# Ameek94/BOBE

Measured on AMD Instinct MI355X. Metric: GP fit+acquisition cycles/sec at N=4096 d=8, 65536 cands; Cholesky GF/s, higher is better.
Workload: dtype f64

## Files before the change

bobe_amd/csrc/gemm_f64.hpp:

```cpp
#pragma once
#include <hip/hip_runtime.h>
#include <stdint.h>
#include <type_traits>

namespace bobe {

typedef double v4d __attribute__((ext_vector_type(4)));
typedef double v2d __attribute__((ext_vector_type(2)));

constexpr int TILE = 128;
constexpr int TK = 16;
constexpr int GEMM_THREADS = 256;

enum Layout { KC = 0, RC = 1 };

template <int L, int R, int BK>
struct Img {
  static constexpr int stride = (L == KC) ? (BK + 2) : (R + 16);
  static constexpr int doubles = (L == KC) ? R * (BK + 2) : BK * (R + 16);
};
constexpr int imax(int a, int b) { return a > b ? a : b; }
template <int TM, int TN, int BK>
constexpr int gemm_smem_doubles() {
  return 2 * (imax(Img<KC, TM, BK>::doubles, Img<RC, TM, BK>::doubles) +
// ... 22 lines not shown
__device__ __forceinline__ void stage_load(v2d (&reg)[R * BK / 512], const double* __restrict__ p, int64_t ld,
                                           int64_t r0, int64_t k0, int t) {
  if (L == KC) {
    constexpr int VPR = BK / 2;
    const int kq = t % VPR;
    const int r = t / VPR;
#pragma unroll
    for (int i = 0; i < R * BK / 512; ++i)
      reg[i] = *reinterpret_cast<const v2d*>(p + (r0 + r + (256 / VPR) * i) * ld + k0 + 2 * kq);
  } else {
    constexpr int VPR = R / 2;
    const int c = t % VPR;
    const int k = t / VPR;
#pragma unroll
    for (int i = 0; i < R * BK / 512; ++i)
      reg[i] = *reinterpret_cast<const v2d*>(p + (k0 + k + (256 / VPR) * i) * ld + r0 + 2 * c);
  }
}

template <int L, int R, int BK>
__device__ __forceinline__ void stage_store(const v2d (&reg)[R * BK / 512], double* img, int t) {
  if (L == KC) {
    constexpr int VPR = BK / 2;
    const int kq = t % VPR;
    const int r = t / VPR;
#pragma unroll
    for (int i = 0; i < R * BK / 512; ++i)
      *reinterpret_cast<v2d*>(img + (r + (256 / VPR) * i) * (BK + 2) + 2 * kq) = reg[i];
  } else {
    constexpr int VPR = R / 2;
    const int c = t % VPR;
    const int k = t / VPR;
#pragma unroll
    for (int i = 0; i < R * BK / 512; ++i)
      *reinterpret_cast<v2d*>(img + (k + (256 / VPR) * i) * (R + 16) + 2 * c) = reg[i];
  }
}

template <int L, int R, int BK>
__device__ __forceinline__ double frag_read(const double* img, int woff, int s, int ks, int lane) {
  if (L == KC)
    return img[(woff + 16 * s + (lane & 15)) * (BK + 2) + 4 * ks + (lane >> 4)];
  else
    return img[(4 * ks + (lane >> 4)) * (R + 16) + woff + 16 * s + (lane & 15)];
}

template <int FM, int FN>
__device__ __forceinline__ void acc_zero(v4d (&acc)[FM][FN]) {
#pragma unroll
  for (int i = 0; i < FM; ++i)
#pragma unroll
    for (int j = 0; j < FN; ++j) acc[i][j] = (v4d){0.0, 0.0, 0.0, 0.0};
}

struct WgSync {
  __device__ __forceinline__ void sync() { __syncthreads(); }
};

template <int LA, int LB, int TM = 128, int TN = 128, int BK = BK128, bool NEGA = false, class SYNC = WgSync, bool TRIL = false>
__device__ __forceinline__ void gemm_tile(v4d (&acc)[TM / 32][TN / 32], const double* __restrict__ A, int64_t lda,
                                          int64_t m0, const double* __restrict__ B, int64_t ldb, int64_t n0,
                                          int64_t kbeg, int64_t kend, double* smem, int tid = threadIdx.x,
                                          SYNC* sy = nullptr) {
  WgSync wg_default;
  constexpr int FM = TM / 32, FN = TN / 32;
  constexpr int IA = Img<LA, TM, BK>::doubles;
  constexpr int IB = Img<LB, TN, BK>::doubles;
  const int t = tid;
  const int lane = t & 63;
  const int wave = t >> 6;
  const int wm = (wave >> 1) * (TM / 2);
  const int wn = (wave & 1) * (TN / 2);
  if (kend <= kbeg) return;
  v2d ra[TM * BK / 512], rb[TN * BK / 512];
  stage_load<LA, TM, BK>(ra, A, lda, m0, kbeg, t);
  stage_load<LB, TN, BK>(rb, B, ldb, n0, kbeg, t);
  stage_store<LA, TM, BK>(ra, smem, t);
  stage_store<LB, TN, BK>(rb, smem + IA, t);
  if (sy) sy->sync(); else wg_default.sync();
  int buf = 0;
  const int wmu = TRIL ? __builtin_amdgcn_readfirstlane(wm) : 0;
  auto kstep = [&](int64_t k0, auto in_c, int rel) {
    constexpr bool IN = decltype(in_c)::value;
    const bool more = (k0 + BK) < kend;
    if (more) {
      stage_load<LA, TM, BK>(ra, A, lda, m0, k0 + BK, t);
      stage_load<LB, TN, BK>(rb, B, ldb, n0, k0 + BK, t);
    }
    const double* ia = smem + buf * (IA + IB);
    const double* ib = ia + IA;
#pragma unroll
    for (int ks = 0; ks < BK / 4; ++ks) {
      double a[FM], b[FN];
#pragma unroll
      for (int s = 0; s < FM; ++s) {
        a[s] = frag_read<LA, TM, BK>(ia, wm, s, ks, lane);
        if (NEGA) a[s] = -a[s];
      }
#pragma unroll
      for (int s = 0; s < FN; ++s) b[s] = frag_read<LB, TN, BK>(ib, wn, s, ks, lane);
#pragma unroll
      for (int i = 0; i < FM; ++i) {
        if (IN && rel + 4 * ks > wmu + 16 * i + 15) continue;
#pragma unroll
        for (int j = 0; j < FN; ++j)
          acc[i][j] = __builtin_amdgcn_mfma_f64_16x16x4f64(a[i], b[j], acc[i][j], 0, 0, 0);
      }
    }
    if (more) {
      double* na = smem + (buf ^ 1) * (IA + IB);
      stage_store<LA, TM, BK>(ra, na, t);
      stage_store<LB, TN, BK>(rb, na + IA, t);
    }
    if (sy) sy->sync(); else wg_default.sync();
    buf ^= 1;
  };
  const int64_t kd = TRIL ? (kend - TM > kbeg ? kend - TM : kbeg) : kend;
  for (int64_t k0 = kbeg; k0 < kd; k0 += BK) kstep(k0, std::false_type(), 0);
  if (TRIL)
    for (int64_t k0 = kd; k0 < kend; k0 += BK) kstep(k0, std::true_type(), (int)(k0 - (kend - TM)));
}

template <int TM = 128>
__device__ __forceinline__ int acc_row(int i, int r, int tid = threadIdx.x) {
  const int t = tid;
  return ((t >> 6) >> 1) * (TM / 2) + 16 * i + ((t & 63) >> 4) + 4 * r;
}
template <int TN = 128>
__device__ __forceinline__ int acc_col(int j, int tid = threadIdx.x) {
  const int t = tid;
  return ((t >> 6) & 1) * (TN / 2) + 16 * j + (t & 15);
}

template <int TM = 128, int TN = 128>
__device__ __forceinline__ void store_tile(const v4d (&acc)[TM / 32][TN / 32], double* __restrict__ C, int64_t ldc,
                                           int64_t m0, int64_t n0, double alpha, double beta, int tid = threadIdx.x) {
#pragma unroll
  for (int i = 0; i < TM / 32; ++i)
#pragma unroll
    for (int j = 0; j < TN / 32; ++j)
#pragma unroll
      for (int r = 0; r < 4; ++r) {
        double* q = C + (m0 + acc_row<TM>(i, r, tid)) * ldc + n0 + acc_col<TN>(j, tid);
        double v = alpha * acc[i][j][r];
        if (beta != 0.0) v += beta * (*q);
        *q = v;
      }
}

template <int TM = 128, int TN = 128>
__device__ __forceinline__ void load_tile(v4d (&acc)[TM / 32][TN / 32], const double* __restrict__ C, int64_t ldc,
                                          int64_t m0, int64_t n0, int tid = threadIdx.x) {
#pragma unroll
  for (int i = 0; i < TM / 32; ++i)
#pragma unroll
    for (int j = 0; j < TN / 32; ++j)
#pragma unroll
      for (int r = 0; r < 4; ++r) acc[i][j][r] = C[(m0 + acc_row<TM>(i, r, tid)) * ldc + n0 + acc_col<TN>(j, tid)];
}

__device__ __forceinline__ void tri_decode(int t, int& i, int& j) {
  int ii = (int)((sqrt(8.0 * (double)t + 1.0) - 1.0) * 0.5);
  while ((ii + 1) * (ii + 2) / 2 <= t) ++ii;
  while (ii * (ii + 1) / 2 > t) --ii;
  i = ii;
  j = t - ii * (ii + 1) / 2;
}

__device__ __forceinline__ int xcd_share(int b, int per) { return per > 0 ? (b & 7) * per + (b >> 3) : b; }

__device__ __forceinline__ void tri_grouped(int t, int n, int& i, int& j) {
  int ii, jj;
  tri_decode(t, ii, jj);
// ... 27 lines not shown
```

bobe_amd/csrc/gp_factor.hip:

```cpp
#include "gp_handle.hpp"

#include <chrono>

#include "chol_kernels.hpp"

using namespace bobe;

namespace bobe {

constexpr int SYRK32_BK = 128, SYRK64_BK = 16;
constexpr int SYRK32_SMEM = gemm_smem_doubles_exact<KC, KC, 32, 32, SYRK32_BK>() * 8 / 2;
constexpr int SYRK64_SMEM = gemm_smem_doubles_exact<KC, KC, 64, 64, SYRK64_BK>() * 8;

void configure_factor_kernels() {
  static bool done[64] = {false};
  int dev = 0;
  HIPCHK(hipGetDevice(&dev));
  if (dev < 0 || dev >= 64 || done[dev]) return;
  allow_big_lds(k_potf2<true>, POTF2_SMEM_BYTES);
  allow_big_lds(k_potf2<false>, POTF2_SMEM_BYTES);
  allow_big_lds(k_trti_diag, POTF2_SMEM_BYTES);
  allow_big_lds(k_trsm_panel, TRSM_SMEM_BYTES);
  allow_big_lds((k_chol_panel<false, 3>), POTF2_SMEM_BYTES);
  allow_big_lds((k_chol_panel<false, 4>), POTF2_SMEM_BYTES);
  allow_big_lds((k_chol_panel<true, 3>), POTF2_SMEM_BYTES);
  allow_big_lds((k_chol_panel<true, 4>), POTF2_SMEM_BYTES);
  allow_big_lds(k_trtri_T<128>, GEMM_SMEM_BYTES);
  allow_big_lds(k_trtri_R<128>, GEMM_SMEM_BYTES);
  allow_big_lds(k_syrk_trail<64, SYRK64_BK>, SYRK64_SMEM);
  allow_big_lds(k_syrk_trail<32, SYRK32_BK>, SYRK32_SMEM);
  allow_big_lds(k_trtri_T<64>, GEMM64_SMEM_BYTES);
  allow_big_lds(k_trtri_R<64>, GEMM64_SMEM_BYTES);
  allow_big_lds(k_trtri_T<32>, GEMM32_SMEM_BYTES);
  allow_big_lds(k_trtri_R<32>, GEMM32_SMEM_BYTES);
  allow_big_lds(k_lauum_tiles32, GEMM32_SMEM_BYTES);
  allow_big_lds(k_lauum_grad<0, 8, 64>, GEMM64_SMEM_BYTES);
  allow_big_lds(k_lauum_grad<0, 16, 64>, GEMM64_SMEM_BYTES);
  allow_big_lds(k_lauum_grad<0, 32, 64>, GEMM64_SMEM_BYTES);
  allow_big_lds(k_lauum_grad<1, 8, 64>, GEMM64_SMEM_BYTES);
  allow_big_lds(k_lauum_grad<1, 16, 64>, GEMM64_SMEM_BYTES);
  allow_big_lds(k_lauum_grad<1, 32, 64>, GEMM64_SMEM_BYTES);
  allow_big_lds(k_lauum_grad<0, 8, 128>, GEMM_SMEM_BYTES);
  allow_big_lds(k_lauum_grad<0, 16, 128>, GEMM_SMEM_BYTES);
  allow_big_lds(k_lauum_grad<0, 32, 128>, GEMM_SMEM_BYTES);
  allow_big_lds(k_lauum_grad<1, 8, 128>, GEMM_SMEM_BYTES);
  allow_big_lds(k_lauum_grad<1, 16, 128>, GEMM_SMEM_BYTES);
  allow_big_lds(k_lauum_grad<1, 32, 128>, GEMM_SMEM_BYTES);
  done[dev] = true;
}

const Tuning& tuning() {
  static Tuning t = [] {
    Tuning v{512, 600, 300, 1, BOBE_MAX_MLL_SLOTS, 2048, 1, 1, false, false, true};
    auto geti = [](const char* name, int& dst) {
      const char* e = std::getenv(name);
      if (e) dst = std::atoi(e);
      return e != nullptr;
    };
    geti("BOBE_SYRK32_BELOW", v.syrk32_below);
    geti("BOBE_TRTRI64", v.trtri64_below);
    geti("BOBE_PAIR_MIN", v.pair_min);
    geti("BOBE_LOCKSTEP_MIN_N", v.lockstep_min_n);
    v.mll_slots_set = geti("BOBE_MLL_SLOTS", v.mll_slots);
    geti("BOBE_GRAPH_MAX_N", v.graph_max_n);
    geti("BOBE_XCD_SHARES", v.xcd_shares);
    geti("BOBE_FILL", v.fill);
    v.trace = std::getenv("BOBE_TRACE") != nullptr;
    int reuse = 1;
    geti("BOBE_FACTOR_REUSE", reuse);
    v.factor_reuse = reuse != 0;
    return v;
  }();
  return t;
}

double default_refine_kappa() {
  static const double v = [] {
    const char* e = std::getenv("BOBE_REFINE_KAPPA");
    return e ? std::atof(e) : 1e6;
  }();
  return v;
}

int default_solve_block() {
  static const int v = [] {
    const char* e = std::getenv("BOBE_SOLVE_BLOCK");
    const int b = e ? std::atoi(e) : TILE;
    return b > 0 ? (b + TILE - 1) / TILE * TILE : TILE;
  }();
  return v;
}

int default_solve_panel() {
  static const int v = [] {
    const char* e = std::getenv("BOBE_SOLVE_PANEL");
    const int b = e ? std::atoi(e) : 512;
    return b > 0 ? (b + TILE - 1) / TILE * TILE : 512;
  }();
  return v;
}

int64_t default_solve_chunk() {
  static const int64_t v = [] {
    const char* e = std::getenv("BOBE_SOLVE_CHUNK");
    const int64_t c = e ? std::atoll(e) : 32768;
    return c > 0 ? (c + TILE - 1) / TILE * TILE : 0;
  }();
  return v;
}

double default_pivot_floor_ulp() {
  static const double v = [] {
    const char* e = std::getenv("BOBE_PIVOT_FLOOR_ULP");
    if (!e) return 0.0;
    const double u = std::atof(e);
    return u >= 0.0 ? u : 0.0;
  }();
  return v;
}

}

void bobe_gp::build_probs() {
// ... 1129 lines not shown
```

bobe_amd/csrc/gp_handle.hpp:

```cpp
#pragma once
#include "../../include/bobe_gp.h"

#include <hip/hip_runtime.h>

#include <algorithm>
#include <array>
#include <climits>
#include <cmath>
#include <cstdio>
#include <cstdlib>
#include <cstring>
#include <map>
#include <mutex>
#include <stdexcept>
#include <string>
#include <vector>

#include "gemm_f64.hpp"
#include "gp_types.hpp"

namespace bobe {

struct Err : std::runtime_error {
  int code;
// ... 12 lines not shown

#define LAUNCH_CHECK() HIPCHK(hipGetLastError())

inline int64_t round_up(int64_t x, int64_t m) { return (x + m - 1) / m * m; }

inline bool is_device_ptr(const void* p) {
  if (!p) return false;
  hipPointerAttribute_t attr;
  hipError_t e = hipPointerGetAttributes(&attr, p);
  if (e != hipSuccess) {
    (void)hipGetLastError();
    return false;
  }
  return attr.type == hipMemoryTypeDevice || attr.type == hipMemoryTypeManaged;
}

struct DBuf {
  void* p = nullptr;
  size_t bytes = 0;
  void ensure(size_t b) {
    if (b <= bytes) return;
    if (p) HIPCHK(hipFree(p));
    p = nullptr;
    bytes = 0;
    HIPCHK(hipMalloc(&p, b));
    bytes = b;
  }
  void release() {
    if (p) (void)hipFree(p);
    p = nullptr;
    bytes = 0;
  }
  double* d() const { return static_cast<double*>(p); }
};

inline double pivot_floor(const Hyper& h, double ulp) {
  const double f = ulp * 2.220446049250313e-16 * (h.kvar + h.noise);
  return f < 0.25 ? f : 0.25;
}
inline bool pivots_resolved(double min_diag, double floor) { return min_diag * min_diag >= floor; }
double default_pivot_floor_ulp();
double default_refine_kappa();
int default_solve_block();
int default_solve_panel();
int64_t default_solve_chunk();

template <typename K>
void allow_big_lds(K kernel, int bytes) {
  HIPCHK(hipFuncSetAttribute(reinterpret_cast<const void*>(kernel), hipFuncAttributeMaxDynamicSharedMemorySize, bytes));
}

struct Tuning {
  int syrk32_below, trtri64_below, pair_min, lockstep_min_n, mll_slots, graph_max_n, xcd_shares, fill;
  bool mll_slots_set, trace, factor_reuse;
};
const Tuning& tuning();

constexpr int LAUUM64_BELOW = 1200;
constexpr int FILL_NEAR = 2;
constexpr int FILL_CHUNK = 3;
constexpr int FILL_SLACK = 16;
constexpr int FILL_PHASE = 1024;

struct TileGrid { int grid, per; };
inline TileGrid tile_grid(int ntiles) {
  if (!tuning().xcd_shares || ntiles < 256) return {ntiles, 0};
  const int per = (ntiles + 7) / 8;
  return {8 * per, per};
}

void configure_factor_kernels();
void configure_sweep_kernels();
void configure_consumer_kernels();

struct Depth { int first, count, nblocks; };

struct EvalTag {
  bool pending = false;
  bool valid = false;
  Hyper h;
  uint64_t gen = 0;
  int64_t Np = 0;
  int info = 0;
  double min_diag = 0.0;
  void arm(const Hyper& hh, uint64_t g, int64_t np) {
    valid = false;
    pending = true;
    h = hh;
    gen = g;
    Np = np;
  }
  void collected(const double* hr) {
    if (!pending) return;
    pending = false;
    valid = true;
    std::memcpy(&info, hr + 100, sizeof(int));
    min_diag = hr[101];
  }
  void clear() { pending = valid = false; }
};
inline bool same_hyper(const Hyper& a, const Hyper& b) {
  if (a.d != b.d || a.kern != b.kern || a.d < 0 || a.d > MAX_D) return false;
  return std::memcmp(a.ls, b.ls, (size_t)a.d * sizeof(double)) == 0 && std::memcmp(&a.kvar, &b.kvar, sizeof(double)) == 0 &&
         std::memcmp(&a.noise, &b.noise, sizeof(double)) == 0;
}

}
// ... 250 lines not shown
```

bobe_amd/csrc/gp_sweep.hip:

```cpp
#include "gp_handle.hpp"

#include "sweep_kernels.hpp"

using namespace bobe;

namespace bobe {
void configure_sweep_kernels() {
  static bool done[64] = {false};
  int dev = 0;
  HIPCHK(hipGetDevice(&dev));
  if (dev < 0 || dev >= 64 || done[dev]) return;
  allow_big_lds(k_trimul, GEMM_SMEM_BYTES);
  allow_big_lds(k_trimul_t, GEMM_SMEM_BYTES);
  allow_big_lds(k_trimul_v64, GEMM64_SMEM_BYTES);
  allow_big_lds(k_trimul_t64, GEMM64_SMEM_BYTES);
  allow_big_lds(k_blk_step, GEMM_SMEM_BYTES);
  allow_big_lds(k_cross_vv<128>, GEMM_SMEM_BYTES);
  allow_big_lds(k_cross_vv<64>, GEMM64_SMEM_BYTES);
  done[dev] = true;
}
}

void bobe_gp::decide_refinement(double min_diag) {
  const double piv = min_diag * min_diag;
  refine_v = refine_kappa >= 0.0 && piv > 0.0 && (hyp.kvar + hyp.noise) / piv > refine_kappa;
}

void bobe_gp::solve_v(double* B, int64_t ldb, int64_t ncp, double* V, int64_t ldv, double* qp, int64_t ldq) {
  if (!refine_v) {
    hipLaunchKernelGGL(k_trimul, dim3((unsigned)(ncp / TILE), (unsigned)nb), dim3(256), GEMM_SMEM_BYTES, stream,
                       (const double*)Linv.d(), Np, nb, (const double*)B, ldb, V, ldv, qp, ldq, (const double*)nullptr,
                       (int64_t)0, 0, (double*)nullptr, (int64_t)0);
    return;
  }
  if (!V) throw Err(BOBE_ERR_STATE, "solve_v: the blocked substitution needs a buffer for V");
  const int bt = std::max(1, solve_block / TILE);
  const int pt = std::max(bt, (int)(solve_panel / TILE) / bt * bt);
  const double* Lf = A.d();
  const double* Li = Linv.d();
  auto step = [&](int u_r0, int u_rows, int u_k0, int u_k1, int s_r0, int s_rows) {
    hipLaunchKernelGGL(k_blk_step, dim3((unsigned)(ncp / TILE), (unsigned)(u_rows + s_rows)), dim3(256), GEMM_SMEM_BYTES,
                       stream, Lf, Li, Np, B, ldb, V, ldv, qp, ldq, u_r0, u_rows, u_k0, u_k1, s_r0, s_rows);
  };
  for (int p0 = 0; p0 < nb; p0 += pt) {
    const int p1 = std::min(nb, p0 + pt);
    if (p0 > 0) step(p0, p1 - p0, 0, p0, 0, 0);
    for (int t0 = p0; t0 < p1; t0 += bt) {
      const int t1 = std::min(p1, t0 + bt);
      step(0, 0, 0, 0, t0, t1 - t0);
      if (t1 < p1) step(t1, p1 - t1, t0, t1, 0, 0);
    }
  }
}

void bobe_gp::prepare_z(const double* Z, int64_t M, int64_t Mp, bool need_w) {
  const bool host_z = !is_device_ptr(Z);
  const bool few = (Mp / TILE) * nb < 2 * std::max(num_cus, 1);
  auto make_w = [&]() {
    if (few)
      hipLaunchKernelGGL(k_trimul_t64, dim3((unsigned)(Mp / 64), (unsigned)(2 * nb)), dim3(256), GEMM64_SMEM_BYTES, stream,
                         (const double*)Linv.d(), Np, 2 * nb, (const double*)VZ.d(), Mp, WZ.d(), Mp);
    else
      hipLaunchKernelGGL(k_trimul_t, dim3((unsigned)(Mp / TILE), (unsigned)nb), dim3(256), GEMM_SMEM_BYTES, stream,
                         (const double*)Linv.d(), Np, nb, (const double*)VZ.d(), Mp, WZ.d(), Mp);
    LAUNCH_CHECK();
    wz_ready = true;
  };
  if (host_z && z_seen_m == M && std::memcmp(z_seen.data(), Z, (size_t)M * d * sizeof(double)) == 0) {
    if (need_w && !wz_ready) make_w();
    return;
  }
  forget_z();
  if (host_z) z_seen.assign(Z, Z + (size_t)M * d);
  const double* zin = fetch(Z, (size_t)M * d, z_stage);
  ZsT.ensure((size_t)d * Mp * sizeof(double));
  kXZ.ensure((size_t)Np * Mp * sizeof(double));
  VZ.ensure((size_t)Np * Mp * sizeof(double));
  WZ.ensure((size_t)Np * Mp * sizeof(double));
  basez.ensure((size_t)Mp * sizeof(double));
  qpart.ensure((size_t)2 * nb * (Mp > chunk ? Mp : chunk) * sizeof(double));
  scale(zin, M, Mp, hyp, ZsT.d(), Mp);
  kernel_matrix_cross(XsT.d(), Np, N, Np, ZsT.d(), Mp, M, Mp, hyp, kXZ.d(), Mp);
  if (refine_v) {
    solve_v(kXZ.d(), Mp, Mp, VZ.d(), Mp, qpart.d(), Mp);
    hipLaunchKernelGGL(k_predict_finalize, dim3((unsigned)((Mp + 255) / 256)), dim3(256), 0, stream,
                       (const double*)qpart.d(), Mp, nb, Mp, hyp.kvar + hyp.noise, 0, basez.d(), (double*)nullptr);
  } else if (few) {
    const int nt = 2 * nb;
    hipLaunchKernelGGL(k_trimul_v64, dim3((unsigned)(Mp / 64), (unsigned)nt), dim3(256), GEMM64_SMEM_BYTES, stream,
                       (const double*)Linv.d(), Np, nt, (const double*)kXZ.d(), Mp, VZ.d(), Mp, qpart.d(), Mp);
    hipLaunchKernelGGL(k_predict_finalize, dim3((unsigned)((Mp + 255) / 256)), dim3(256), 0, stream,
                       (const double*)qpart.d(), Mp, nt, Mp, hyp.kvar + hyp.noise, 0, basez.d(), (double*)nullptr);
  } else {
    hipLaunchKernelGGL(k_trimul, dim3((unsigned)(Mp / TILE), (unsigned)nb), dim3(256), GEMM_SMEM_BYTES, stream,
                       (const double*)Linv.d(), Np, nb, (const double*)kXZ.d(), Mp, VZ.d(), Mp, qpart.d(), Mp,
                       (const double*)nullptr, (int64_t)0, 0, (double*)nullptr, (int64_t)0);
    hipLaunchKernelGGL(k_predict_finalize, dim3((unsigned)((Mp + 255) / 256)), dim3(256), 0, stream,
                       (const double*)qpart.d(), Mp, nb, Mp, hyp.kvar + hyp.noise, 0, basez.d(), (double*)nullptr);
  }
  LAUNCH_CHECK();
  if (need_w) make_w();
  if (host_z) z_seen_m = M;
}

void bobe_gp::sweep(const double* cand, int64_t C, const double* Z, int64_t M, double y_std, double* wipv,
                    double* wipstd, double* mean, double* var, int policy, int64_t* argmin_v, double* min_v,
                    int64_t* argmin_s, double* min_s, double* fantasy_out, bool gated) {
  if (!factored) throw Err(BOBE_ERR_STATE, "call bobe_gp_factor first");
  if (C <= 0) throw Err(BOBE_ERR_ARG, "C must be positive");
  const bool do_wip = (Z != nullptr);
  if (do_wip && M <= 0) throw Err(BOBE_ERR_ARG, "M must be positive");
  const int64_t Mp = do_wip ? round_up(M, TILE) : 0;
  const int nzt = (int)(Mp / TILE);
  const double kself = hyp.kvar + hyp.noise;
  const bool need_v = wipv || argmin_v || min_v;
  const bool need_s = wipstd || argmin_s || min_s;
  const double* cin = fetch(cand, (size_t)C * d, in_stage);
  if (do_wip) prepare_z(Z, M, Mp, false);
  const int64_t CH = (refine_v && solve_chunk > 0 && !chunk_set) ? solve_chunk : chunk;
  bool cand_is_z = false;
  if (do_wip && C == M && C <= CH && !mean && !var) {
    if (is_device_ptr(cand) || is_device_ptr(Z)) cand_is_z = (cand == Z);
    else cand_is_z = std::memcmp(cand, Z, (size_t)C * d * sizeof(double)) == 0;
  }
  const int64_t SC = round_up(std::min<int64_t>(C, std::max<int64_t>(CH, 65536)), CH);
  CsT.ensure((size_t)d * SC * sizeof(double));
  if (!cand_is_z) kXC.ensure((size_t)Np * CH * sizeof(double));
  sc.ensure((size_t)SC * sizeof(double));
  qpart.ensure((size_t)nb * (Mp > CH ? Mp : CH) * sizeof(double));
  part.ensure((size_t)nb * (Np > CH ? Np : CH) * sizeof(double));
  if (do_wip) pv.ensure((size_t)Mp * SC * sizeof(double));
  if ((do_wip || refine_v) && !cand_is_z) vxc.ensure((size_t)Np * CH * sizeof(double));
  const bool fuse_cross = do_wip && !refine_v && C > CH;
  if (fuse_cross) vxc2.ensure((size_t)Np * CH * sizeof(double));
  double* vbuf[2] = {vxc.d(), fuse_cross ? vxc2.d() : vxc.d()};
  int vsel = 0;
  struct { bool valid; const double* V; int64_t ncp; double* cross; } pend = {false, nullptr, 0, nullptr};
  auto cross_alone = [&](const double* Vc, int64_t ncp_, double* cross_out, int64_t ldvc) {
    prof_begin(BOBE_PROF_CROSSVV);
    if ((int64_t)nzt * (ncp_ / TILE) >= 2 * std::max(num_cus, 1))
      hipLaunchKernelGGL(k_cross_vv<128>, dim3((unsigned)(ncp_ / TILE), (unsigned)nzt), dim3(256), GEMM_SMEM_BYTES, stream,
                         (const double*)VZ.d(), Mp, Vc, ldvc, Np, cross_out, SC);
    else
      hipLaunchKernelGGL(k_cross_vv<64>, dim3((unsigned)(ncp_ / 64), (unsigned)(Mp / 64)), dim3(256), GEMM64_SMEM_BYTES,
                         stream, (const double*)VZ.d(), Mp, Vc, ldvc, Np, cross_out, SC);
    prof_end(BOBE_PROF_CROSSVV);
  };
  double* d_mean = out_dev(mean, C, o_mean);
  double* d_var = out_dev(var, C, o_var);
  double* d_wipv = nullptr;
  double* d_wipstd = nullptr;
  if (do_wip) {
    if (need_v) {
      if (wipv) d_wipv = out_dev(wipv, C, o_wipv);
      else { o_wipv.ensure(C * sizeof(double)); d_wipv = o_wipv.d(); }
    }
    if (need_s) {
      if (wipstd) d_wipstd = out_dev(wipstd, C, o_wipstd);
      else { o_wipstd.ensure(C * sizeof(double)); d_wipstd = o_wipstd.d(); }
    }
  }
  double* d_fant = nullptr;
  if (fantasy_out) {
    d_fant = is_device_ptr(fantasy_out) ? fantasy_out : (kout.ensure((size_t)C * M * sizeof(double)), kout.d());
  }
  const int dcap = d <= 8 ? 8 : (d <= 16 ? 16 : 32);
  for (int64_t s0 = 0; s0 < C; s0 += SC) {
    const int64_t ns = (C - s0 < SC) ? (C - s0) : SC;
    const int64_t nsp = round_up(ns, TILE);
    scale(cin + s0 * d, ns, nsp, hyp, CsT.d(), SC);
    for (int64_t c0 = 0; c0 < ns; c0 += CH) {
      const int64_t nc = (ns - c0 < CH) ? (ns - c0) : CH;
      const int64_t ncp = round_up(nc, TILE);
      if (cand_is_z) {
        hipLaunchKernelGGL(k_colsq_tile_parts, dim3((unsigned)((ncp + 255) / 256), (unsigned)nb), dim3(256), 0, stream,
                           (const double*)VZ.d(), Mp, ncp, qpart.d(), CH);
        cross_alone(VZ.d(), ncp, pv.d() + c0, Mp);
        hipLaunchKernelGGL(k_predict_finalize, dim3((unsigned)((nc + 255) / 256)), dim3(256), 0, stream,
                           (const double*)qpart.d(), CH, nb, nc, kself, policy, sc.d() + c0, (double*)nullptr);
        LAUNCH_CHECK();
        continue;
      }
      prof_begin(BOBE_PROF_KXC);
      kernel_matrix_cross(XsT.d(), Np, N, Np, CsT.d() + c0, SC, nc, ncp, hyp, kXC.d(), CH,
                          d_mean ? (const double*)alpha.d() : nullptr, d_mean ? part.d() : nullptr, CH);
      prof_end(BOBE_PROF_KXC);
      if (d_mean) {
        hipLaunchKernelGGL(k_colsum_parts, dim3((unsigned)((nc + 255) / 256)), dim3(256), 0, stream,
                           (const double*)part.d(), CH, nb, 0, nc, d_mean + s0 + c0);
      }
      if (do_wip || d_var) {
        double* vcur = vbuf[vsel];
        prof_begin(BOBE_PROF_TRIMUL);
        if (fuse_cross) {
          const int ncv = (int)(ncp / TILE), ncx = pend.valid ? (int)(pend.ncp / TILE) : 0;
          const int nz = pend.valid ? nzt : 0;
          hipLaunchKernelGGL(k_trimul, dim3((unsigned)std::max(ncv, ncx), (unsigned)(nb + nz)), dim3(256), GEMM_SMEM_BYTES,
                             stream, (const double*)Linv.d(), Np, nb, (const double*)kXC.d(), CH, vcur, CH, qpart.d(), CH,
                             (const double*)VZ.d(), Mp, nz, pend.cross, SC, pend.V, CH, ncx, ncv);
          pend = {true, vcur, ncp, pv.d() + c0};
          vsel ^= 1;
        } else {
          solve_v(kXC.d(), CH, ncp, (do_wip || refine_v) ? vcur : nullptr, CH, qpart.d(), CH);
        }
        prof_end(BOBE_PROF_TRIMUL);
        if (do_wip && !fuse_cross) cross_alone(vcur, ncp, pv.d() + c0, CH);
        hipLaunchKernelGGL(k_predict_finalize, dim3((unsigned)((nc + 255) / 256)), dim3(256), 0, stream,
                           (const double*)qpart.d(), CH, nb, nc, kself, policy, sc.d() + c0,
                           d_var ? d_var + s0 + c0 : nullptr);
      }
      LAUNCH_CHECK();
    }
    if (pend.valid) {
      cross_alone(pend.V, pend.ncp, pend.cross, CH);
      pend.valid = false;
    }
    if (do_wip) {
      const dim3 grid((unsigned)((ns + 63) / 64));
      const size_t sm = (size_t)(d + 1) * 128 * sizeof(double);
      double* vo = d_fant ? d_fant + s0 * M : nullptr;
      prof_begin(BOBE_PROF_CROSS);
#define WS(KE, DC)                                                                                              \
  hipLaunchKernelGGL((k_wip_score<KE, DC>), grid, dim3(256), sm, stream, (const double*)pv.d(), SC,             \
                     (const double*)CsT.d(), SC, (const double*)ZsT.d(), Mp, M, (const double*)sc.d(),          \
                     (const double*)basez.d(), ns, hyp, y_std * y_std, d_wipv ? d_wipv + s0 : nullptr,          \
                     d_wipstd ? d_wipstd + s0 : nullptr, vo, M)
      if (hyp.kern == 0) {
        if (dcap == 8) WS(0, 8); else if (dcap == 16) WS(0, 16); else WS(0, 32);
      } else {
        if (dcap == 8) WS(1, 8); else if (dcap == 16) WS(1, 16); else WS(1, 32);
      }
#undef WS
      prof_end(BOBE_PROF_CROSS);
      LAUNCH_CHECK();
    }
  }
  if (gated && gate_on(gate) && (d_mean || d_var)) gate_apply(cin, C, nullptr, nullptr, d_mean, d_var, nullptr, nullptr);
  o_misc.ensure(8 * sizeof(double));
  double* m_val = o_misc.d();
  int64_t* m_idx = reinterpret_cast<int64_t*>(o_misc.d() + 2);
  const bool want_v = do_wip && (argmin_v || min_v);
  const bool want_s = do_wip && (argmin_s || min_s);
  if (want_v) hipLaunchKernelGGL(k_argmin, dim3(1), dim3(1024), 0, stream, (const double*)d_wipv, C, m_val, m_idx);
  if (want_s)
    hipLaunchKernelGGL(k_argmin, dim3(1), dim3(1024), 0, stream, (const double*)d_wipstd, C, m_val + 1, m_idx + 1);
  LAUNCH_CHECK();
  out_finish(mean, C, o_mean);
  out_finish(var, C, o_var);
  if (do_wip) {
    out_finish(wipv, C, o_wipv);
// ... 380 lines not shown
```

bobe_amd/csrc/sweep_kernels.hpp:

```cpp
#pragma once
#include "kernels_common.hpp"

namespace bobe {

__global__ __launch_bounds__(256, 2) void k_trimul(const double* __restrict__ Linv, int64_t ldi, int nb,
                                                   const double* __restrict__ B, int64_t ldb, double* __restrict__ V,
                                                   int64_t ldv, double* __restrict__ qpart, int64_t ldq,
                                                   const double* __restrict__ VZ, int64_t ldw, int nzt,
                                                   double* __restrict__ crossT, int64_t ldx,
                                                   const double* __restrict__ Bx = nullptr, int64_t ldbx = 0, int ncx = 0,
                                                   int ncv = 1 << 30) {
  extern __shared__ double smem[];
  const int tc = blockIdx.x;
  v4d acc[4][4];
  acc_zero(acc);
  if ((int)blockIdx.y < nzt) {
    if (tc >= ncx) return;
    const int tz = blockIdx.y;
    gemm_tile<RC, RC>(acc, VZ, ldw, (int64_t)tz * TILE, Bx, ldbx, (int64_t)tc * TILE, 0, (int64_t)nb * TILE, smem);
    store_tile(acc, crossT, ldx, (int64_t)tz * TILE, (int64_t)tc * TILE, 1.0, 0.0);
    return;
  }
  if (tc >= ncv) return;
  const int ti = nb - 1 - ((int)blockIdx.y - nzt);
  gemm_tile<KC, RC, TILE, TILE, BK128, false, WgSync, true>(acc, Linv, ldi, (int64_t)ti * TILE, B, ldb, (int64_t)tc * TILE, 0,
                                                            (int64_t)(ti + 1) * TILE, smem);
  if (V) store_tile(acc, V, ldv, (int64_t)ti * TILE, (int64_t)tc * TILE, 1.0, 0.0);
  if (qpart) {
    const int t = threadIdx.x, lane = t & 63, wave = t >> 6;
    double* red = smem;
#pragma unroll
    for (int j = 0; j < 4; ++j) {
      double s = 0.0;
#pragma unroll
      for (int i = 0; i < 4; ++i)
#pragma unroll
        for (int r = 0; r < 4; ++r) s += acc[i][j][r] * acc[i][j][r];
      s += __shfl_xor(s, 16, 64);
      s += __shfl_xor(s, 32, 64);
      if (lane < 16) red[(wave >> 1) * TILE + (wave & 1) * 64 + 16 * j + lane] = s;
    }
    __syncthreads();
    if (t < TILE) qpart[(int64_t)ti * ldq + (int64_t)tc * TILE + t] = red[t] + red[TILE + t];
  }
}

__global__ __launch_bounds__(256, 2) void k_blk_step(const double* __restrict__ L, const double* __restrict__ Linv,
                                                     int64_t ld, double* __restrict__ B, int64_t ldb,
                                                     double* __restrict__ V, int64_t ldv, double* __restrict__ qpart,
                                                     int64_t ldq, int u_r0, int u_rows, int u_k0, int u_k1, int s_r0,
                                                     int s_rows) {
  extern __shared__ double smem[];
  const int tc = blockIdx.x;
  v4d acc[4][4];
  acc_zero(acc);
  if ((int)blockIdx.y < u_rows) {
    const int ti = u_r0 + (int)blockIdx.y;
    gemm_tile<KC, RC>(acc, L, ld, (int64_t)ti * TILE, V, ldv, (int64_t)tc * TILE, (int64_t)u_k0 * TILE,
                      (int64_t)u_k1 * TILE, smem);
    store_tile(acc, B, ldb, (int64_t)ti * TILE, (int64_t)tc * TILE, -1.0, 1.0);
    return;
  }
  const int ti = s_r0 + s_rows - 1 - ((int)blockIdx.y - u_rows);
  gemm_tile<KC, RC, TILE, TILE, BK128, false, WgSync, true>(acc, Linv, ld, (int64_t)ti * TILE, B, ldb, (int64_t)tc * TILE,
                                                            (int64_t)s_r0 * TILE, (int64_t)(ti + 1) * TILE, smem);
  store_tile(acc, V, ldv, (int64_t)ti * TILE, (int64_t)tc * TILE, 1.0, 0.0);
  if (qpart) {
    const int t = threadIdx.x, lane = t & 63, wave = t >> 6;
    double* red = smem;
#pragma unroll
    for (int j = 0; j < 4; ++j) {
      double s = 0.0;
#pragma unroll
      for (int i = 0; i < 4; ++i)
#pragma unroll
        for (int r = 0; r < 4; ++r) s += acc[i][j][r] * acc[i][j][r];
      s += __shfl_xor(s, 16, 64);
      s += __shfl_xor(s, 32, 64);
      if (lane < 16) red[(wave >> 1) * TILE + (wave & 1) * 64 + 16 * j + lane] = s;
    }
    __syncthreads();
    if (t < TILE) qpart[(int64_t)ti * ldq + (int64_t)tc * TILE + t] = red[t] + red[TILE + t];
  }
}

__global__ void k_vec_axpy(double* __restrict__ y, const double* __restrict__ a, const double* __restrict__ b, double sb,
                           int64_t n) {
  const int64_t i = (int64_t)blockIdx.x * blockDim.x + threadIdx.x;
  if (i < n) y[i] = a[i] + sb * b[i];
}

__global__ __launch_bounds__(256) void k_colsq_tile_parts(const double* __restrict__ V, int64_t ldv, int64_t ncols,
                                                          double* __restrict__ qpart, int64_t ldq) {
  const int64_t c = (int64_t)blockIdx.x * 256 + threadIdx.x;
  const int ti = blockIdx.y;
  if (c >= ncols) return;
  const double* col = V + ((int64_t)ti * TILE) * ldv + c;
  double half[2];
#pragma unroll
  for (int h = 0; h < 2; ++h) {
    double sq[4];
#pragma unroll
    for (int q = 0; q < 4; ++q) {
      double s = 0.0;
#pragma unroll
      for (int i = 0; i < 4; ++i)
#pragma unroll
        for (int r = 0; r < 4; ++r) {
          const double v = col[(int64_t)(64 * h + 16 * i + q + 4 * r) * ldv];
          s += v * v;
        }
      sq[q] = s;
    }
    half[h] = (sq[0] + sq[1]) + (sq[2] + sq[3]);
  }
  qpart[(int64_t)ti * ldq + c] = half[0] + half[1];
}

template <int T>
__global__ __launch_bounds__(256, 2) void k_cross_vv(const double* __restrict__ VZ, int64_t ldz,
                                                     const double* __restrict__ V, int64_t ldv, int64_t kend,
                                                     double* __restrict__ crossT, int64_t ldx) {
  extern __shared__ double smem[];
  const int tc = blockIdx.x, tz = blockIdx.y;
  v4d acc[T / 32][T / 32];
  acc_zero(acc);
  if constexpr (T == 128) {
    gemm_tile<RC, RC>(acc, VZ, ldz, (int64_t)tz * TILE, V, ldv, (int64_t)tc * TILE, 0, kend, smem);
    store_tile(acc, crossT, ldx, (int64_t)tz * TILE, (int64_t)tc * TILE, 1.0, 0.0);
  } else {
    gemm_tile<RC, RC, 64, 64, BK64>(acc, VZ, ldz, (int64_t)tz * 64, V, ldv, (int64_t)tc * 64, 0, kend, smem);
    store_tile<64, 64>(acc, crossT, ldx, (int64_t)tz * 64, (int64_t)tc * 64, 1.0, 0.0);
  }
}

__global__ __launch_bounds__(256, 2) void k_trimul_t(const double* __restrict__ Linv, int64_t ldi, int nb,
                                                  const double* __restrict__ V, int64_t ldv, double* __restrict__ W,
                                                  int64_t ldw) {
  extern __shared__ double smem[];
  const int ti = blockIdx.y;
  const int tc = blockIdx.x;
  v4d acc[4][4];
  acc_zero(acc);
  gemm_tile<RC, RC>(acc, Linv, ldi, (int64_t)ti * TILE, V, ldv, (int64_t)tc * TILE, (int64_t)ti * TILE,
                    (int64_t)nb * TILE, smem);
  store_tile(acc, W, ldw, (int64_t)ti * TILE, (int64_t)tc * TILE, 1.0, 0.0);
}

__global__ __launch_bounds__(256, 2) void k_trimul_v64(const double* __restrict__ Linv, int64_t ldi, int nt,
                                                       const double* __restrict__ B, int64_t ldb, double* __restrict__ V,
                                                       int64_t ldv, double* __restrict__ qpart, int64_t ldq) {
  extern __shared__ double smem[];
  const int tc = blockIdx.x;
  const int ti = nt - 1 - (int)blockIdx.y;
  v4d acc[2][2];
  acc_zero(acc);
  gemm_tile<KC, RC, 64, 64, BK64>(acc, Linv, ldi, (int64_t)ti * 64, B, ldb, (int64_t)tc * 64, 0, (int64_t)(ti + 1) * 64, smem);
  store_tile<64, 64>(acc, V, ldv, (int64_t)ti * 64, (int64_t)tc * 64, 1.0, 0.0);
  const int t = threadIdx.x, lane = t & 63, wave = t >> 6;
  double* red = smem;
#pragma unroll
  for (int j = 0; j < 2; ++j) {
    double s = 0.0;
#pragma unroll
    for (int i = 0; i < 2; ++i)
#pragma unroll
      for (int r = 0; r < 4; ++r) s += acc[i][j][r] * acc[i][j][r];
    s += __shfl_xor(s, 16, 64);
    s += __shfl_xor(s, 32, 64);
    if (lane < 16) red[(wave >> 1) * 64 + (wave & 1) * 32 + 16 * j + lane] = s;
  }
  __syncthreads();
  if (t < 64) qpart[(int64_t)ti * ldq + (int64_t)tc * 64 + t] = red[t] + red[64 + t];
}

__global__ __launch_bounds__(256, 2) void k_trimul_t64(const double* __restrict__ Linv, int64_t ldi, int nt,
                                                       const double* __restrict__ V, int64_t ldv, double* __restrict__ W,
                                                       int64_t ldw) {
  extern __shared__ double smem[];
  const int ti = blockIdx.y;
  const int tc = blockIdx.x;
// ... 643 lines not shown
```

Measured before the change: 18.45.

## Stage 128-tile GEMM operands via buffer_load_lds with swizzle and fragment double-buffering

Adds a 128x128 f64 GEMM tile path that loads global data straight into LDS with buffer_load...lds, skipping the register staging round trip. It also uses an XOR-swizzled KC layout without padding and prefetches the next k-slice's fragments while the current MFMAs run. The new path is the default for k_trimul and k_cross_vv<128>, and an env var falls back to the old path. It also adds optional s_memtime instrumentation behind a compile flag. Risks: each kstep issues a redundant stage even when there are no more k-slices, the swizzle is new correctness surface, and LDS occupancy changes.

```diff
diff --git a/bobe_amd/csrc/gemm_f64.hpp b/bobe_amd/csrc/gemm_f64.hpp
--- a/bobe_amd/csrc/gemm_f64.hpp
+++ b/bobe_amd/csrc/gemm_f64.hpp
@@ -98,6 +98,62 @@
 #pragma unroll
     for (int j = 0; j < FN; ++j) acc[i][j] = (v4d){0.0, 0.0, 0.0, 0.0};
 }
+
+#ifdef BOBE_GEMM_STAMPS
+__device__ unsigned long long* g_stamps;
+__device__ __forceinline__ unsigned long long stamp_time() {
+  unsigned long long t;
+  __builtin_amdgcn_sched_barrier(0);
+  asm volatile("s_memtime %0\n\ts_waitcnt lgkmcnt(0)" : "=s"(t)::"memory");
+  __builtin_amdgcn_sched_barrier(0);
+  return t;
+}
+__device__ __forceinline__ unsigned long long stamp_real() {
+  unsigned long long t;
+  __builtin_amdgcn_sched_barrier(0);
+  asm volatile("s_memrealtime %0\n\ts_waitcnt lgkmcnt(0)" : "=s"(t)::"memory");
+  __builtin_amdgcn_sched_barrier(0);
+  return t;
+}
+struct Stamps {
+  unsigned long long t0, r0, last, seg[4], steps;
+  __device__ __forceinline__ void begin() {
+    r0 = stamp_real();
+    t0 = last = stamp_time();
+    seg[0] = seg[1] = seg[2] = seg[3] = steps = 0;
+  }
+  __device__ __forceinline__ void mark(int i) {
+    const unsigned long long t = stamp_time();
+    seg[i] += t - last;
+    last = t;
+  }
+  __device__ __forceinline__ void end(int tid) {
+    const unsigned long long t1 = stamp_time(), r1 = stamp_real();
+    if ((tid & 63) == 0 && g_stamps) {
+      unsigned long long* o = g_stamps + ((blockIdx.y * gridDim.x + blockIdx.x) * 4 + (tid >> 6)) * 8;
+      o[0] = t1 - t0;
+      o[1] = r1 - r0;
+      o[2] = seg[0];
+      o[3] = seg[1];
+      o[4] = seg[2];
+      o[5] = seg[3];
+      o[6] = steps;
+      o[7] = 1;
+    }
+  }
+};
+#define BOBE_STAMPS_DECL Stamps st_; st_.begin();
+#define BOBE_STAMP(i) st_.mark(i)
+#define BOBE_STAMP_STEP() (++st_.steps)
+#define BOBE_STAMP_VMWAIT() asm volatile("s_waitcnt vmcnt(0)" ::: "memory")
+#define BOBE_STAMPS_END(tid) st_.end(tid)
+#else
+#define BOBE_STAMPS_DECL
+#define BOBE_STAMP(i)
+#define BOBE_STAMP_STEP()
+#define BOBE_STAMP_VMWAIT()
+#define BOBE_STAMPS_END(tid)
+#endif
 
 struct WgSync {
   __device__ __forceinline__ void sync() { __syncthreads(); }
@@ -124,6 +180,7 @@
   stage_store<LA, TM, BK>(ra, smem, t);
   stage_store<LB, TN, BK>(rb, smem + IA, t);
   if (sy) sy->sync(); else wg_default.sync();
+  BOBE_STAMPS_DECL
   int buf = 0;
   const int wmu = TRIL ? __builtin_amdgcn_readfirstlane(wm) : 0;
   auto kstep = [&](int64_t k0, auto in_c, int rel) {
@@ -145,6 +202,7 @@
       }
 #pragma unroll
       for (int s = 0; s < FN; ++s) b[s] = frag_read<LB, TN, BK>(ib, wn, s, ks, lane);
+      if (ks == 0) BOBE_STAMP(0);
 #pragma unroll
       for (int i = 0; i < FM; ++i) {
         if (IN && rel + 4 * ks > wmu + 16 * i + 15) continue;
@@ -153,18 +211,138 @@
           acc[i][j] = __builtin_amdgcn_mfma_f64_16x16x4f64(a[i], b[j], acc[i][j], 0, 0, 0);
       }
     }
+    BOBE_STAMP(1);
     if (more) {
       double* na = smem + (buf ^ 1) * (IA + IB);
       stage_store<LA, TM, BK>(ra, na, t);
       stage_store<LB, TN, BK>(rb, na + IA, t);
     }
+    BOBE_STAMP(2);
     if (sy) sy->sync(); else wg_default.sync();
+    BOBE_STAMP(3);
+    BOBE_STAMP_STEP();
     buf ^= 1;
   };
   const int64_t kd = TRIL ? (kend - TM > kbeg ? kend - TM : kbeg) : kend;
   for (int64_t k0 = kbeg; k0 < kd; k0 += BK) kstep(k0, std::false_type(), 0);
   if (TRIL)
     for (int64_t k0 = kd; k0 < kend; k0 += BK) kstep(k0, std::true_type(), (int)(k0 - (kend - TM)));
+  BOBE_STAMPS_END(t);
+}
+
+template <int L>
+struct Img128 {
+  static constexpr int doubles = (L == KC) ? 128 * 16 : 16 * (128 + 16);
+};
+template <int LA, int LB>
+constexpr int gemm128_smem_doubles() { return 2 * (Img128<LA>::doubles + Img128<LB>::doubles); }
+static_assert(gemm128_smem_doubles<RC, RC>() <= GEMM_SMEM_DOUBLES && gemm128_smem_doubles<KC, RC>() <= GEMM_SMEM_DOUBLES,
+              "the 128-tile LDS images must fit the launches' GEMM_SMEM_BYTES");
+
+template <int L>
+__device__ __forceinline__ void glds_stage128(const double* __restrict__ p, int64_t ld, int64_t r0, int64_t k0, double* img,
+                                              int wave, int lane) {
+  const double* base = (L == KC) ? p + r0 * ld + k0 : p + k0 * ld + r0;
+  const __amdgpu_buffer_rsrc_t rs = __builtin_amdgcn_make_buffer_rsrc((void*)base, 0, 0x7fffffff, 0x00020000);
+#pragma unroll
+  for (int i = 0; i < 4; ++i) {
+    const int g = wave + 4 * i;
+    unsigned off;
+    double* dst;
+    if (L == KC) {
+      const int r = 8 * g + (lane >> 3);
+      off = (unsigned)((r * ld + 2 * ((lane & 7) ^ ((r >> 1) & 7))) * 8);
+      dst = img + 128 * g;
+    } else {
+      off = (unsigned)((g * ld + 2 * lane) * 8);
+      dst = img + (128 + 16) * g;
+    }
+    __builtin_amdgcn_raw_ptr_buffer_load_lds(rs, (__attribute__((address_space(3))) void*)dst, 16, off, 0, 0, 0);
+  }
+}
+
+template <int L>
+__device__ __forceinline__ double frag_read128(const double* img, int woff, int s, int ks, int lane) {
+  if (L == KC) {
+    const int h = (lane >> 5) ^ ((lane & 15) >> 1);
+    return img[(woff + 16 * s + (lane & 15)) * 16 + 2 * ((2 * ks) ^ h) + ((lane >> 4) & 1)];
+  } else {
+    return img[(4 * ks + (lane >> 4)) * (128 + 16) + woff + 16 * s + (lane & 15)];
+  }
+}
+
+template <int LA, int LB, bool NEGA = false, bool TRIL = false>
+__device__ __forceinline__ void gemm_tile128_glds(v4d (&acc)[4][4], const double* __restrict__ A, int64_t lda, int64_t m0,
+                                                  const double* __restrict__ B, int64_t ldb, int64_t n0, int64_t kbeg,
+                                                  int64_t kend, double* smem, int tid = threadIdx.x) {
+  constexpr int BK = 16, TM = 128;
+  constexpr int IA = Img128<LA>::doubles, IB = Img128<LB>::doubles;
+  const int lane = tid & 63;
+  const int wave = __builtin_amdgcn_readfirstlane(tid >> 6);
+  const int wm = (wave >> 1) * 64;
+  const int wn = (wave & 1) * 64;
+  if (kend <= kbeg) return;
+  auto stage = [&](int64_t k0, int b) {
+    double* ia = smem + b * (IA + IB);
+    glds_stage128<LA>(A, lda, m0, k0, ia, wave, lane);
+    glds_stage128<LB>(B, ldb, n0, k0, ia + IA, wave, lane);
+  };
+  double fa[2][4], fb[2][4];
+  auto frags = [&](double (&a)[4], double (&b)[4], const double* ia, int ks) {
+#pragma unroll
+    for (int s = 0; s < 4; ++s) {
+      a[s] = frag_read128<LA>(ia, wm, s, ks, lane);
+      if (NEGA) a[s] = -a[s];
+    }
+#pragma unroll
+    for (int s = 0; s < 4; ++s) b[s] = frag_read128<LB>(ia + IA, wn, s, ks, lane);
+  };
+  stage(kbeg, 0);
+  __syncthreads();
+  BOBE_STAMPS_DECL
+  frags(fa[0], fb[0], smem, 0);
+  BOBE_STAMP(0);
+  int buf = 0;
+  auto kstep = [&](int64_t k0, auto in_c, int rel) {
+    constexpr bool IN = decltype(in_c)::value;
+    const bool more = (k0 + BK) < kend;
+    auto mfmas = [&](int ks) {
+      const double(&a)[4] = fa[ks & 1];
+      const double(&b)[4] = fb[ks & 1];
+#pragma unroll
+      for (int i = 0; i < 4; ++i) {
+        if (IN && rel + 4 * ks > wm + 16 * i + 15) continue;
+#pragma unroll
+        for (int j = 0; j < 4; ++j) acc[i][j] = __builtin_amdgcn_mfma_f64_16x16x4f64(a[i], b[j], acc[i][j], 0, 0, 0);
+      }
+    };
+    stage(more ? k0 + BK : k0, buf ^ 1);
+    const double* ia = smem + buf * (IA + IB);
+#pragma unroll
+    for (int ks = 0; ks < BK / 4 - 1; ++ks) {
+      frags(fa[(ks + 1) & 1], fb[(ks + 1) & 1], ia, ks + 1);
+      __builtin_amdgcn_sched_barrier(0);
+      mfmas(ks);
+      __builtin_amdgcn_sched_barrier(0);
+    }
+    BOBE_STAMP(1);
+    BOBE_STAMP_VMWAIT();
+    BOBE_STAMP(2);
+    __syncthreads();
+    BOBE_STAMP(3);
+    BOBE_STAMP_STEP();
+    buf ^= 1;
+    frags(fa[0], fb[0], smem + buf * (IA + IB), 0);
+    __builtin_amdgcn_sched_barrier(0);
+    mfmas(BK / 4 - 1);
+    __builtin_amdgcn_sched_barrier(0);
+    BOBE_STAMP(0);
+  };
+  const int64_t kd = TRIL ? (kend - TM > kbeg ? kend - TM : kbeg) : kend;
+  for (int64_t k0 = kbeg; k0 < kd; k0 += BK) kstep(k0, std::false_type(), 0);
+  if (TRIL)
+    for (int64_t k0 = kd; k0 < kend; k0 += BK) kstep(k0, std::true_type(), (int)(k0 - (kend - TM)));
+  BOBE_STAMPS_END(tid);
 }
 
 template <int TM = 128>
diff --git a/bobe_amd/csrc/gp_factor.hip b/bobe_amd/csrc/gp_factor.hip
--- a/bobe_amd/csrc/gp_factor.hip
+++ b/bobe_amd/csrc/gp_factor.hip
@@ -51,7 +51,7 @@
 
 const Tuning& tuning() {
   static Tuning t = [] {
-    Tuning v{512, 600, 300, 1, BOBE_MAX_MLL_SLOTS, 2048, 1, 1, false, false, true};
+    Tuning v{512, 600, 300, 1, BOBE_MAX_MLL_SLOTS, 2048, 1, 1, false, false, true, true};
     auto geti = [](const char* name, int& dst) {
       const char* e = std::getenv(name);
       if (e) dst = std::atoi(e);
@@ -69,6 +69,9 @@
     int reuse = 1;
     geti("BOBE_FACTOR_REUSE", reuse);
     v.factor_reuse = reuse != 0;
+    int glds = 1;
+    geti("BOBE_GEMM_GLDS", glds);
+    v.gemm_glds = glds != 0;
     return v;
   }();
   return t;
diff --git a/bobe_amd/csrc/gp_handle.hpp b/bobe_amd/csrc/gp_handle.hpp
--- a/bobe_amd/csrc/gp_handle.hpp
+++ b/bobe_amd/csrc/gp_handle.hpp
@@ -88,7 +88,7 @@
 
 struct Tuning {
   int syrk32_below, trtri64_below, pair_min, lockstep_min_n, mll_slots, graph_max_n, xcd_shares, fill;
-  bool mll_slots_set, trace, factor_reuse;
+  bool mll_slots_set, trace, factor_reuse, gemm_glds;
 };
 const Tuning& tuning();
 
diff --git a/bobe_amd/csrc/gp_sweep.hip b/bobe_amd/csrc/gp_sweep.hip
--- a/bobe_amd/csrc/gp_sweep.hip
+++ b/bobe_amd/csrc/gp_sweep.hip
@@ -10,15 +10,20 @@
   int dev = 0;
   HIPCHK(hipGetDevice(&dev));
   if (dev < 0 || dev >= 64 || done[dev]) return;
-  allow_big_lds(k_trimul, GEMM_SMEM_BYTES);
+  allow_big_lds(k_trimul<true>, GEMM_SMEM_BYTES);
+  allow_big_lds(k_trimul<false>, GEMM_SMEM_BYTES);
   allow_big_lds(k_trimul_t, GEMM_SMEM_BYTES);
   allow_big_lds(k_trimul_v64, GEMM64_SMEM_BYTES);
   allow_big_lds(k_trimul_t64, GEMM64_SMEM_BYTES);
   allow_big_lds(k_blk_step, GEMM_SMEM_BYTES);
-  allow_big_lds(k_cross_vv<128>, GEMM_SMEM_BYTES);
+  allow_big_lds(k_cross_vv<128, true>, GEMM_SMEM_BYTES);
+  allow_big_lds(k_cross_vv<128, false>, GEMM_SMEM_BYTES);
   allow_big_lds(k_cross_vv<64>, GEMM64_SMEM_BYTES);
   done[dev] = true;
 }
+
+static auto trimul_kernel() { return tuning().gemm_glds ? k_trimul<true> : k_trimul<false>; }
+static auto cross_vv128_kernel() { return tuning().gemm_glds ? k_cross_vv<128, true> : k_cross_vv<128, false>; }
 }
 
 void bobe_gp::decide_refinement(double min_diag) {
@@ -28,9 +33,9 @@
 
 void bobe_gp::solve_v(double* B, int64_t ldb, int64_t ncp, double* V, int64_t ldv, double* qp, int64_t ldq) {
   if (!refine_v) {
-    hipLaunchKernelGGL(k_trimul, dim3((unsigned)(ncp / TILE), (unsigned)nb), dim3(256), GEMM_SMEM_BYTES, stream,
+    hipLaunchKernelGGL(trimul_kernel(), dim3((unsigned)(ncp / TILE), (unsigned)nb), dim3(256), GEMM_SMEM_BYTES, stream,
                        (const double*)Linv.d(), Np, nb, (const double*)B, ldb, V, ldv, qp, ldq, (const double*)nullptr,
-                       (int64_t)0, 0, (double*)nullptr, (int64_t)0);
+                       (int64_t)0, 0, (double*)nullptr, (int64_t)0, (const double*)nullptr, (int64_t)0, 0, 1 << 30);
     return;
   }
   if (!V) throw Err(BOBE_ERR_STATE, "solve_v: the blocked substitution needs a buffer for V");
@@ -92,9 +97,10 @@
     hipLaunchKernelGGL(k_predict_finalize, dim3((unsigned)((Mp + 255) / 256)), dim3(256), 0, stream,
                        (const double*)qpart.d(), Mp, nt, Mp, hyp.kvar + hyp.noise, 0, basez.d(), (double*)nullptr);
   } else {
-    hipLaunchKernelGGL(k_trimul, dim3((unsigned)(Mp / TILE), (unsigned)nb), dim3(256), GEMM_SMEM_BYTES, stream,
+    hipLaunchKernelGGL(trimul_kernel(), dim3((unsigned)(Mp / TILE), (unsigned)nb), dim3(256), GEMM_SMEM_BYTES, stream,
                        (const double*)Linv.d(), Np, nb, (const double*)kXZ.d(), Mp, VZ.d(), Mp, qpart.d(), Mp,
-                       (const double*)nullptr, (int64_t)0, 0, (double*)nullptr, (int64_t)0);
+                       (const double*)nullptr, (int64_t)0, 0, (double*)nullptr, (int64_t)0, (const double*)nullptr,
+                       (int64_t)0, 0, 1 << 30);
     hipLaunchKernelGGL(k_predict_finalize, dim3((unsigned)((Mp + 255) / 256)), dim3(256), 0, stream,
                        (const double*)qpart.d(), Mp, nb, Mp, hyp.kvar + hyp.noise, 0, basez.d(), (double*)nullptr);
   }
@@ -139,7 +145,7 @@
   auto cross_alone = [&](const double* Vc, int64_t ncp_, double* cross_out, int64_t ldvc) {
     prof_begin(BOBE_PROF_CROSSVV);
     if ((int64_t)nzt * (ncp_ / TILE) >= 2 * std::max(num_cus, 1))
-      hipLaunchKernelGGL(k_cross_vv<128>, dim3((unsigned)(ncp_ / TILE), (unsigned)nzt), dim3(256), GEMM_SMEM_BYTES, stream,
+      hipLaunchKernelGGL(cross_vv128_kernel(), dim3((unsigned)(ncp_ / TILE), (unsigned)nzt), dim3(256), GEMM_SMEM_BYTES, stream,
                          (const double*)VZ.d(), Mp, Vc, ldvc, Np, cross_out, SC);
     else
       hipLaunchKernelGGL(k_cross_vv<64>, dim3((unsigned)(ncp_ / 64), (unsigned)(Mp / 64)), dim3(256), GEMM64_SMEM_BYTES,
@@ -195,7 +201,7 @@
         if (fuse_cross) {
           const int ncv = (int)(ncp / TILE), ncx = pend.valid ? (int)(pend.ncp / TILE) : 0;
           const int nz = pend.valid ? nzt : 0;
-          hipLaunchKernelGGL(k_trimul, dim3((unsigned)std::max(ncv, ncx), (unsigned)(nb + nz)), dim3(256), GEMM_SMEM_BYTES,
+          hipLaunchKernelGGL(trimul_kernel(), dim3((unsigned)std::max(ncv, ncx), (unsigned)(nb + nz)), dim3(256), GEMM_SMEM_BYTES,
                              stream, (const double*)Linv.d(), Np, nb, (const double*)kXC.d(), CH, vcur, CH, qpart.d(), CH,
                              (const double*)VZ.d(), Mp, nz, pend.cross, SC, pend.V, CH, ncx, ncv);
           pend = {true, vcur, ncp, pv.d() + c0};
diff --git a/bobe_amd/csrc/sweep_kernels.hpp b/bobe_amd/csrc/sweep_kernels.hpp
--- a/bobe_amd/csrc/sweep_kernels.hpp
+++ b/bobe_amd/csrc/sweep_kernels.hpp
@@ -3,6 +3,7 @@
 
 namespace bobe {
 
+template <bool GLDS>
 __global__ __launch_bounds__(256, 2) void k_trimul(const double* __restrict__ Linv, int64_t ldi, int nb,
                                                    const double* __restrict__ B, int64_t ldb, double* __restrict__ V,
                                                    int64_t ldv, double* __restrict__ qpart, int64_t ldq,
@@ -17,14 +18,21 @@
   if ((int)blockIdx.y < nzt) {
     if (tc >= ncx) return;
     const int tz = blockIdx.y;
-    gemm_tile<RC, RC>(acc, VZ, ldw, (int64_t)tz * TILE, Bx, ldbx, (int64_t)tc * TILE, 0, (int64_t)nb * TILE, smem);
+    if constexpr (GLDS)
+      gemm_tile128_glds<RC, RC>(acc, VZ, ldw, (int64_t)tz * TILE, Bx, ldbx, (int64_t)tc * TILE, 0, (int64_t)nb * TILE, smem);
+    else
+      gemm_tile<RC, RC>(acc, VZ, ldw, (int64_t)tz * TILE, Bx, ldbx, (int64_t)tc * TILE, 0, (int64_t)nb * TILE, smem);
     store_tile(acc, crossT, ldx, (int64_t)tz * TILE, (int64_t)tc * TILE, 1.0, 0.0);
     return;
   }
   if (tc >= ncv) return;
   const int ti = nb - 1 - ((int)blockIdx.y - nzt);
-  gemm_tile<KC, RC, TILE, TILE, BK128, false, WgSync, true>(acc, Linv, ldi, (int64_t)ti * TILE, B, ldb, (int64_t)tc * TILE, 0,
-                                                            (int64_t)(ti + 1) * TILE, smem);
+  if constexpr (GLDS)
+    gemm_tile128_glds<KC, RC, false, true>(acc, Linv, ldi, (int64_t)ti * TILE, B, ldb, (int64_t)tc * TILE, 0,
+                                           (int64_t)(ti + 1) * TILE, smem);
+  else
+    gemm_tile<KC, RC, TILE, TILE, BK128, false, WgSync, true>(acc, Linv, ldi, (int64_t)ti * TILE, B, ldb, (int64_t)tc * TILE,
+                                                              0, (int64_t)(ti + 1) * TILE, smem);
   if (V) store_tile(acc, V, ldv, (int64_t)ti * TILE, (int64_t)tc * TILE, 1.0, 0.0);
   if (qpart) {
     const int t = threadIdx.x, lane = t & 63, wave = t >> 6;
@@ -117,7 +125,7 @@
   qpart[(int64_t)ti * ldq + c] = half[0] + half[1];
 }
 
-template <int T>
+template <int T, bool GLDS = false>
 __global__ __launch_bounds__(256, 2) void k_cross_vv(const double* __restrict__ VZ, int64_t ldz,
                                                      const double* __restrict__ V, int64_t ldv, int64_t kend,
                                                      double* __restrict__ crossT, int64_t ldx) {
@@ -126,7 +134,10 @@
   v4d acc[T / 32][T / 32];
   acc_zero(acc);
   if constexpr (T == 128) {
-    gemm_tile<RC, RC>(acc, VZ, ldz, (int64_t)tz * TILE, V, ldv, (int64_t)tc * TILE, 0, kend, smem);
+    if constexpr (GLDS)
+      gemm_tile128_glds<RC, RC>(acc, VZ, ldz, (int64_t)tz * TILE, V, ldv, (int64_t)tc * TILE, 0, kend, smem);
+    else
+      gemm_tile<RC, RC>(acc, VZ, ldz, (int64_t)tz * TILE, V, ldv, (int64_t)tc * TILE, 0, kend, smem);
     store_tile(acc, crossT, ldx, (int64_t)tz * TILE, (int64_t)tc * TILE, 1.0, 0.0);
   } else {
     gemm_tile<RC, RC, 64, 64, BK64>(acc, VZ, ldz, (int64_t)tz * 64, V, ldv, (int64_t)tc * 64, 0, kend, smem);
```

Measured after the change: 19.06 (median of 6 runs). 1.03x the previous value.
